# chenhonghua/MVIP-NeRF

Hardware: AMD Instinct MI355X
Metric: rays_per_sec (coarse+fine, 64+128 samples, 504x378) (higher is better)
Workload: dtype f32; 1 GPU; render 378x504 frame, 64 coarse + 128 fine samples, 8x256 MLP x2, lindisp, white_bkgd, test-mode kwargs (BASELINE configs[1] geometry at the metric resolution); points_per_ray=192, chunk=32768, parallelism=rays x1 (whole frames on one GPU)

## Files before the change

### include/mvip_nerf.h

```cpp
#ifndef MVIP_NERF_H
#define MVIP_NERF_H

#include <stdint.h>

#ifdef __cplusplus
extern "C" {
#endif

#define MVIP_OK        0
#define MVIP_EINVAL   -1
#define MVIP_ELAUNCH  -2
#define MVIP_EUNSUP   -3

#define MVIP_ABI_VERSION 5

int         mvip_abi_version(void);
int         mvip_build_is_experiment(void);
const char *mvip_strerror(int code);
const char *mvip_last_hip_error(void);
int         mvip_device_info(int *n_cu, int *lds_bytes, char *arch_out, int arch_cap);

int mvip_get_rays(const float *c2w, int H, int W, float focal, int y0, int x0, int h, int w,
                  float *rays_o, float *rays_d, void *stream);

// ... 24 lines not shown
                                      float *raw, void *stream);
int mvip_mlp_forward_rays_stash_f16x3_w16(const float *image, const float *rows, const float *z, int64_t B, int S,
                                          float *raw, float *stash, void *stream);

int mvip_mlp_forward_rays(const float *packed, const float *rows, const float *z, int64_t B, int S,
                          float *raw, int precision, void *stream);

int mvip_mlp_forward_points(const float *packed, const float *pts, const float *dirs, int64_t P,
                            float *raw, int precision, void *stream);

int mvip_mlp_pack16(const float *const *params_host, const float *packed, float *packed16, void *stream);
int mvip_mlp_forward_rays16(const float *packed16, const float *rows, const float *z, int64_t B, int S,
                            float *raw, void *stream);
int mvip_mlp_forward_points16(const float *packed16, const float *pts, const float *dirs, int64_t P,
                              float *raw, void *stream);
int mvip_mlp_encode16_probe(const float *pts, const float *dirs, int64_t P, float *out_old, float *out_new, void *stream);

int64_t mvip_mlp_packed_fold_floats(void);
int mvip_mlp_fold_pack16(const float *const *params_host, float *packed16_ext, void *stream);
int mvip_mlp_forward_rays16_fold(const float *packed16_ext, const float *rows, const float *z, int64_t B, int S,
                                 float *raw, void *stream);
int mvip_mlp_forward_points16_fold(const float *packed16_ext, const float *pts, const float *dirs, int64_t P,
                                   float *raw, void *stream);

int mvip_render_coarse_fused(const float *packed16, const float *rows, int64_t B, const float *t_vals, int lindisp,
                             const float *t_rand, const float *noise, const float *u, int u_is_row, int Nf, int flags,
                             float *rgb0, float *disp0, float *acc0, float *depth0, float *weights0, float *alpha0,
                             float *z_merged, float *z_std, void *stream);
int mvip_render_fine_fused(const float *packed16, const float *rows, const float *z, int64_t B, const float *noise,
                           int flags, float *raw, float *rgb, float *disp, float *acc, float *depth, float *weights,
                           float *alpha, void *stream);
int mvip_render_coarse_fused_fold(const float *packed16_ext, const float *rows, int64_t B, const float *t_vals, int lindisp,
                                  const float *t_rand, const float *noise, const float *u, int u_is_row, int Nf, int flags,
                                  float *rgb0, float *disp0, float *acc0, float *depth0, float *weights0, float *alpha0,
                                  float *z_merged, float *z_std, void *stream);
int mvip_render_fine_fused_fold(const float *packed16_ext, const float *rows, const float *z, int64_t B, const float *noise,
                                int flags, float *raw, float *rgb, float *disp, float *acc, float *depth, float *weights,
                                float *alpha, void *stream);

int64_t mvip_mlp_backward_workspace_bytes(int64_t tile_points);
int mvip_mlp_backward_rays(const float *packed, const float *rows, const float *z, int64_t B, int S,
                           const float *d_raw, float *const *grads_host, void *workspace,
                           int64_t tile_points, int precision, void *stream);
int mvip_mlp_backward_points(const float *packed, const float *pts, const float *dirs, int64_t P,
                             const float *d_raw, float *const *grads_host, void *workspace,
                             int64_t tile_points, int precision, void *stream);
int64_t mvip_mlp_stash_floats(int64_t P);
int mvip_mlp_forward_rays_stash(const float *packed, const float *rows, const float *z, int64_t B,
                                int S, float *raw, float *stash, int precision, void *stream);
int mvip_mlp_forward_points_stash(const float *packed, const float *pts, const float *dirs, int64_t P,
                                  float *raw, float *stash, int precision, void *stream);
int mvip_mlp_forward_rays_stash16(const float *packed16, const float *rows, const float *z, int64_t B, int S,
                                  float *raw, float *stash, void *stream);
int mvip_mlp_backward_stash(const float *packed, const float *stash, int64_t P, const float *d_raw,
                            float *const *grads_host, void *workspace, int64_t tile_points,
                            int precision, void *stream);
int mvip_mlp_unpack_grads(const float *grad_packed, float *const *grads_host, int accumulate,
                          void *stream);

#define MVIP_COMP_WHITE   1
#define MVIP_COMP_DETACHW 2
// ... 255 lines not shown
```

### mvip_nerf_amd/_lib.py

```python
import ctypes
import os

import torch

_HERE = os.path.dirname(os.path.abspath(__file__))
LIB_PATH = os.environ.get('MVIP_LIB_PATH') or os.path.join(_HERE, 'lib', 'libmvipnerf.so')

_c_f = ctypes.c_void_p
_i64 = ctypes.c_int64
_int = ctypes.c_int
_flt = ctypes.c_float

_SIGNATURES = {
    'mvip_abi_version': (_int, []),
    'mvip_build_is_experiment': (_int, []),
    'mvip_strerror': (ctypes.c_char_p, [_int]),
    'mvip_last_hip_error': (ctypes.c_char_p, []),
    'mvip_device_info': (_int, [ctypes.POINTER(_int), ctypes.POINTER(_int), ctypes.c_char_p, _int]),
    'mvip_get_rays': (_int, [_c_f, _int, _int, _flt, _int, _int, _int, _int, _c_f, _c_f, _c_f]),
    'mvip_ray_rows': (_int, [_c_f, _c_f, _c_f, _flt, _flt, _i64, _c_f, _c_f]),
    'mvip_ray_rows_from_pose': (_int, [_c_f, _int, _int, _flt, _flt, _flt, _c_f, _i64, _c_f, _c_f]),
    'mvip_stratified_z': (_int, [_c_f, _int, _i64, _int, _c_f, _int, _c_f, _c_f, _c_f]),
    'mvip_posenc': (_int, [_c_f, _i64, _int, _c_f, _c_f]),
    'mvip_mlp_packed_floats': (_i64, []),
# ... 2 lines not shown
    'mvip_mlp_forward_rays_f16x3': (_int, [_c_f, _c_f, _c_f, _i64, _int, _c_f, _c_f]),
    'mvip_mlp_forward_points_f16x3': (_int, [_c_f, _c_f, _c_f, _i64, _c_f, _c_f]),
    'mvip_mlp_pack_f16x3_w16': (_int, [ctypes.POINTER(ctypes.c_void_p), _c_f, _c_f, _c_f]),
    'mvip_mlp_forward_rays_f16x3_w16': (_int, [_c_f, _c_f, _c_f, _i64, _int, _c_f, _c_f]),
    'mvip_mlp_forward_points_f16x3_w16': (_int, [_c_f, _c_f, _c_f, _i64, _c_f, _c_f]),
    'mvip_mlp_forward_rays_stash_f16x3_w16': (_int, [_c_f, _c_f, _c_f, _i64, _int, _c_f, _c_f, _c_f]),
    'mvip_mlp_forward_rays': (_int, [_c_f, _c_f, _c_f, _i64, _int, _c_f, _int, _c_f]),
    'mvip_mlp_forward_points': (_int, [_c_f, _c_f, _c_f, _i64, _c_f, _int, _c_f]),
    'mvip_mlp_pack16': (_int, [ctypes.POINTER(ctypes.c_void_p), _c_f, _c_f, _c_f]),
    'mvip_mlp_forward_rays16': (_int, [_c_f, _c_f, _c_f, _i64, _int, _c_f, _c_f]),
    'mvip_mlp_forward_rays_stash16': (_int, [_c_f, _c_f, _c_f, _i64, _int, _c_f, _c_f, _c_f]),
    'mvip_mlp_forward_points16': (_int, [_c_f, _c_f, _c_f, _i64, _c_f, _c_f]),
    'mvip_mlp_encode16_probe': (_int, [_c_f, _c_f, _i64, _c_f, _c_f, _c_f]),
    'mvip_render_coarse_fused': (_int, [_c_f, _c_f, _i64, _c_f, _int, _c_f, _c_f, _c_f, _int, _int, _int, _c_f, _c_f, _c_f, _c_f,
                                        _c_f, _c_f, _c_f, _c_f, _c_f]),
    'mvip_render_fine_fused': (_int, [_c_f, _c_f, _c_f, _i64, _c_f, _int, _c_f, _c_f, _c_f, _c_f, _c_f, _c_f, _c_f, _c_f]),
    'mvip_mlp_packed_fold_floats': (_i64, []),
    'mvip_mlp_fold_pack16': (_int, [ctypes.POINTER(ctypes.c_void_p), _c_f, _c_f]),
    'mvip_mlp_forward_rays16_fold': (_int, [_c_f, _c_f, _c_f, _i64, _int, _c_f, _c_f]),
    'mvip_mlp_forward_points16_fold': (_int, [_c_f, _c_f, _c_f, _i64, _c_f, _c_f]),
    'mvip_render_coarse_fused_fold': (_int, [_c_f, _c_f, _i64, _c_f, _int, _c_f, _c_f, _c_f, _int, _int, _int, _c_f, _c_f, _c_f,
                                             _c_f, _c_f, _c_f, _c_f, _c_f, _c_f]),
    'mvip_render_fine_fused_fold': (_int, [_c_f, _c_f, _c_f, _i64, _c_f, _int, _c_f, _c_f, _c_f, _c_f, _c_f, _c_f, _c_f, _c_f]),
    'mvip_mlp_backward_workspace_bytes': (_i64, [_i64]),
    'mvip_mlp_backward_rays': (_int, [_c_f, _c_f, _c_f, _i64, _int, _c_f, ctypes.POINTER(ctypes.c_void_p), _c_f, _i64,
                                      _int, _c_f]),
    'mvip_mlp_backward_points': (_int, [_c_f, _c_f, _c_f, _i64, _c_f, ctypes.POINTER(ctypes.c_void_p), _c_f, _i64, _int,
                                        _c_f]),
    'mvip_mlp_stash_floats': (_i64, [_i64]),
    'mvip_mlp_forward_rays_stash': (_int, [_c_f, _c_f, _c_f, _i64, _int, _c_f, _c_f, _int, _c_f]),
    'mvip_mlp_forward_points_stash': (_int, [_c_f, _c_f, _c_f, _i64, _c_f, _c_f, _int, _c_f]),
    'mvip_mlp_backward_stash': (_int, [_c_f, _c_f, _i64, _c_f, ctypes.POINTER(ctypes.c_void_p), _c_f, _i64, _int, _c_f]),
    'mvip_mlp_unpack_grads': (_int, [_c_f, ctypes.POINTER(ctypes.c_void_p), _int, _c_f]),
    'mvip_composite_forward': (_int, [_c_f, _c_f, _c_f, _int, _c_f, _i64, _int, _int, _c_f, _c_f, _c_f, _c_f,
                                      _c_f, _c_f, _c_f]),
    'mvip_composite_backward': (_int, [_c_f, _c_f, _c_f, _int, _c_f, _i64, _int, _int, _c_f, _c_f, _c_f, _c_f,
                                       _c_f, _c_f, _c_f, _c_f]),
    'mvip_sample_pdf_merge': (_int, [_c_f, _c_f, _c_f, _int, _i64, _int, _int, _c_f, _c_f, _c_f, _c_f, _c_f,
                                     _c_f]),
    'mvip_sample_pdf': (_int, [_c_f, _c_f, _c_f, _int, _i64, _int, _int, _c_f, _c_f, _c_f, _c_f]),
    'mvip_depth2xyz': (_int, [_c_f, _int, _int, _flt, _flt, _flt, _flt, _c_f, _c_f]),
    'mvip_depth2xyz_backward': (_int, [_c_f, _int, _int, _flt, _flt, _flt, _flt, _c_f, _c_f]),
    'mvip_normal_fit_forward': (_int, [_c_f, _int, _int, _int, _c_f, _c_f, _c_f, _c_f]),
    'mvip_normal_fit_backward': (_int, [_c_f, _c_f, _c_f, _c_f, _int, _int, _int, _c_f, _c_f, _c_f]),
    'mvip_sds_add_noise': (_int, [_c_f, _c_f, _flt, _flt, _i64, _c_f, _c_f]),
    'mvip_sds_grad': (_int, [_c_f, _c_f, _c_f, _flt, _flt, _i64, _int, _c_f, _c_f]),
# ... 187 lines not shown
```

### mvip_nerf_amd/csrc/build.py

```python
import hashlib
import os
import shutil
import subprocess
import sys
from concurrent.futures import ThreadPoolExecutor

HERE = os.path.dirname(os.path.abspath(__file__))
PKG = os.path.dirname(HERE)
EXTRA_FLAGS = os.environ.get('MVIP_EXTRA_FLAGS', '').split()
EXPERIMENT = any(f.startswith('-DMVIP_EXPERIMENT') for f in EXTRA_FLAGS)
LIB_DIR = os.path.join(PKG, 'lib_experiment' if EXPERIMENT else 'lib')
OBJ_DIR = os.path.join(LIB_DIR, 'obj')
LIB_PATH = os.path.join(LIB_DIR, 'libmvipnerf.so')

SOURCES = ['api.hip', 'rays.hip', 'composite.hip', 'sample_pdf.hip', 'mlp_pack.hip', 'mlp_fwd.hip', 'mlp_fwd16.hip', 'mlp_fwd16_fold.hip', 'mlp_encode16_probe.hip', 'mlp_fwd_f16x3.hip', 'mlp_fwd16_f16x3.hip',
           'mlp_bwd.hip', 'mlp_bwd16.hip', 'mlp_bwd_f16x3.hip', 'normal_fit.hip', 'sds_elem.hip', 'group_norm.hip', 'conv3x3.hip', 'attention.hip', 'transformer.hip', 'hashgrid.hip', 'hashgrid_fused.hip', 'skinny_gemm.hip',
           'sd_sample.hip', 'mcubes.hip', 'occupancy.hip', 'region.hip', 'distortion.hip', 'harmonic.hip', 'warp.hip', 'ssim.hip', 'components.hip']
FLAGS = ['--offload-arch=gfx950', '-O3', '-std=c++17', '-fPIC', '-ffp-contract=off', '-Wall',
         '-Wno-unused-function'] + EXTRA_FLAGS


def _hipcc():
    for c in (os.environ.get('HIPCC'), shutil.which('hipcc'), '/opt/rocm/bin/hipcc'):
        if c and os.path.exists(c):
            return c
    raise RuntimeError('hipcc not found (need ROCm with gfx950 support)')


def _headers():
    hs = [os.path.join(HERE, f) for f in sorted(os.listdir(HERE)) if f.endswith('.h')]
    hs.append(os.path.join(os.path.dirname(PKG), 'include', 'mvip_nerf.h'))
    return hs


def _digest(path, header_blob):
    h = hashlib.sha256()
    h.update(open(path, 'rb').read())
    h.update(header_blob)
# ... 46 lines not shown
```

### mvip_nerf_amd/csrc/mlp_device16.h

```cpp
#pragma once
#include "common.h"
#include "mlp_layout.h"
#include "mlp_device.h"
#include <type_traits>

namespace mvip {
using namespace mlp;

namespace f16p {

typedef float f32x4 __attribute__((ext_vector_type(4)));
template <int V> using ic = std::integral_constant<int, V>;
template <int N, class F, int I = 0>
__device__ __forceinline__ void static_for(F &&f) {
    if constexpr (I < N) { f(ic<I>{}); static_for<N, F, I + 1>(static_cast<F &&>(f)); }
}

template <int C>
__device__ __forceinline__ float enc_channel(float x, float y, float z, int c) {
    const int m = c >= 3 ? c - 3 : 0;
    const int oct = m / 6, rem = m - 6 * oct;
    const int d = rem >= 3 ? rem - 3 : rem;
    const int dsel = c < 3 ? c : d;
    const float xv = dsel == 0 ? x : (dsel == 1 ? y : z);
// ... 47 lines not shown
    for (int t = 0; t < 4; ++t) emb[t] = ld4(row + (((4 * t + g) ^ n) << 2));
    __builtin_amdgcn_wave_barrier();
    row = stage + n * 32;
    const int nd = n >> 1;
    auto at_d = [&](int c) -> float & { return row[(((c >> 2) ^ nd) << 2) + (c & 3)]; };
    at_d(g < 3 ? g : 27) = g == 0 ? vx : (g == 1 ? vy : (g == 2 ? vz : 0.f));
    at_d(28 + g) = 0.f;
#pragma unroll
    for (int k = 0; k < 3; ++k) {
        const int j = g + 4 * k;
        const int oct = j / 3, axis = j - 3 * oct;
        const float xv = axis == 0 ? vx : (axis == 1 ? vy : vz);
        float s, c;
        sincosf(xv * __int_as_float((127 + oct) << 23), &s, &c);
        at_d(3 + 6 * oct + axis) = s;
        at_d(6 + 6 * oct + axis) = c;
    }
    __builtin_amdgcn_wave_barrier();
#pragma unroll
    for (int t = 0; t < 2; ++t) edir[t] = ld4(row + (((4 * t + g) ^ nd) << 2));
    __builtin_amdgcn_wave_barrier();
}

template <int NSLOT = NSLOT16, bool WRAP = false, bool FOLD = false>
struct Stream16T {
    const float *packed;
    float *lds;
    int wave, lane;
    int total_chunks = FOLD ? FOLD_TOTAL_CHUNKS : TOTAL_CHUNKS;
    lds_cfloat *lds_read = nullptr;
    static constexpr int nslot = NSLOT;
    static constexpr bool wrap = WRAP;
    __device__ __forceinline__ void issue_chunk(int g, int slot) const {
        if (WRAP && g >= total_chunks) g -= total_chunks;
        if (g < total_chunks) {
            const float *src = packed + (int64_t)g * CHUNK_FLOATS + wave * 512 + lane * 4;
            if constexpr (FOLD) { if (g >= FOLD_FIRST_CHUNK) src += FOLD_TAIL_A - FOLD_FIRST_CHUNK * CHUNK_FLOATS; }
            float *dst = lds + slot * CHUNK_FLOATS + wave * 512;
            glds<0>(src, dst);
            glds<1024>(src, dst);
        }
    }
    template <int BI>
    __device__ __forceinline__ f32x4 read_block() const {
        constexpr int off = ((BI / CHUNK_BLOCKS) % NSLOT) * CHUNK_FLOATS + (BI % CHUNK_BLOCKS) * BLOCK_FLOATS;
        if constexpr (WRAP) return ld4(lds_read + off + lane * 4);
        else return ld4(lds + off + lane * 4);
    }
};
using Stream16 = Stream16T<>;

__device__ __forceinline__ f32x4 mfma4(float a, float b, f32x4 c) {
    return __builtin_amdgcn_mfma_f32_16x16x4f32(a, b, c, 0, 0, 0);
}

struct NoPre16 { template <class T> __device__ __forceinline__ int operator()(T) const { return 0; } };
template <int BASE, int NTO, int NTI, bool LAST, bool HASB, class St, class Bias, class BSrc, class Pre, class Epi>
__device__ __forceinline__ void layer16x(const St &st, f32x4 &a, Bias bias, BSrc bsrc, Pre pre, Epi epi) {
    using PV = decltype(pre(ic<0>{}));
    f32x4 accs[2];
    PV pvs[2];
    static_for<NTO>([&](auto to_) {
        constexpr int TO = decltype(to_)::value;
        f32x4 &acc = accs[TO & 1];
        pvs[TO & 1] = pre(to_);
        if constexpr (HASB) acc = ld4(bias + 16 * TO + 4 * (st.lane >> 4));
        else acc = f32x4{0.f, 0.f, 0.f, 0.f};
        static_for<NTI>([&](auto ti_) {
            constexpr int TI = decltype(ti_)::value;
            constexpr int bi = BASE + TO * NTI + TI;
            constexpr bool last_block = LAST && (TO == NTO - 1) && (TI == NTI - 1);
            if constexpr (bi % CHUNK_BLOCKS == 0) st.issue_chunk(bi / CHUNK_BLOCKS + 2, (bi / CHUNK_BLOCKS + 2) % St::nslot);
            const f32x4 b = bsrc(ti_);
            acc = mfma4(a[0], b[0], acc);
            __builtin_amdgcn_sched_barrier(0);
            f32x4 an = a;
            if constexpr (!last_block) an = st.template read_block<bi + 1>();
            else if constexpr (St::wrap) an = st.template read_block<0>();
            __builtin_amdgcn_sched_barrier(0);
            acc = mfma4(a[1], b[1], acc);
            acc = mfma4(a[2], b[2], acc);
            acc = mfma4(a[3], b[3], acc);
            if constexpr (TI == NTI - 1) asm volatile("" : "+v"(acc));
#ifndef MVIP_EXPERIMENT_NO_BARRIER
            if constexpr (bi % CHUNK_BLOCKS == CHUNK_BLOCKS - 1) __syncthreads();
#endif
            a = an;
            if constexpr (TO > 0 && TI == 1) epi(ic<TO - 1>{}, accs[(TO - 1) & 1], pvs[(TO - 1) & 1]);
        });
    });
    epi(ic<NTO - 1>{}, accs[(NTO - 1) & 1], pvs[(NTO - 1) & 1]);
}
template <int BASE, int NTO, int NTI, bool LAST, class St, class Bias, class BSrc, class Epi>
__device__ __forceinline__ void layer16(const St &st, f32x4 &a, Bias bias, BSrc bsrc, Epi epi) {
    layer16x<BASE, NTO, NTI, LAST, true>(st, a, bias, bsrc, NoPre16{}, [&](auto to, const f32x4 &acc, int) { epi(to, acc); });
}

template <bool RELU>
__device__ __forceinline__ f32x4 act16(const f32x4 &acc) {
#ifdef MVIP_EXPERIMENT_NO_EPILOGUE
    return acc;
#endif
    f32x4 r;
#pragma unroll
    for (int i = 0; i < 4; ++i) {
        float v = acc[i];
        if (RELU) {
            const int bits = __builtin_bit_cast(int, v);
// ... 10 lines not shown
```

### mvip_nerf_amd/csrc/mlp_fwd16_kernel.h

```cpp
#pragma once
#include <stdlib.h>
#include "mlp_device16.h"
#include "rays_device.h"
#include "composite_device.h"
#include "sample_pdf_device.h"


namespace mvip {
using namespace mlp;

namespace f16p {

struct FuseArgs {
    const float *t_vals, *t_rand, *noise, *u;
    int u_is_row, lindisp, flags, Nf;
    float *rgb, *disp, *acc, *depth, *weights, *alpha, *z_merged, *z_std;
};

template <bool FROM_RAYS, bool STASH = false, int FUSE = 0, bool FOLD = false>
__global__ void __launch_bounds__(512, 2)
mlp_forward16_kernel(const float *__restrict__ packed, const float *__restrict__ in_a, const float *__restrict__ in_b,
                     int64_t P, int S, float *__restrict__ raw, float *__restrict__ stash = nullptr, int64_t n_pt = 0,
                     const FuseArgs fa = FuseArgs{}) {
    static_assert(!(STASH && FOLD), "the stash-writing forward needs the feature activations: it cannot fold");
    constexpr int NCHUNK = FOLD ? FOLD_TOTAL_CHUNKS : TOTAL_CHUNKS;
    __shared__ __attribute__((aligned(16))) float lds[LDS16_FLOATS];
    float *raw_s = lds + ((NCHUNK - 2) % NSLOT16) * CHUNK_FLOATS;
    const int lane = threadIdx.x & 63;
    const int wave = __builtin_amdgcn_readfirstlane(threadIdx.x >> 6);
    const int n = lane & 15, g = lane >> 4;
    int64_t p = (int64_t)blockIdx.x * WG_POINTS + wave * 16 + n;
    const bool live = p < P;
    if (!live) p = P - 1;

    Stream16T<NSLOT16, false, FOLD> st{packed, lds, wave, lane};
    constexpr int SEC_B_AT = FOLD ? FOLD_TAIL_B : SEC_A_FLOATS;
    for (int b = wave; b < SEC_B_FLOATS / BLOCK_FLOATS; b += 8)
        glds<0>(packed + SEC_B_AT + b * BLOCK_FLOATS + lane * 4, lds + RING16_FLOATS + b * BLOCK_FLOATS);
    st.issue_chunk(0, 0);
    st.issue_chunk(1, 1);

    float px, py, pz, vx, vy, vz;
    float zz = 0.f, zn = 0.f, nz = 0.f, dnorm = 0.f, tail_u = 2.f;
    int s_idx = 0;
    if constexpr (FROM_RAYS) {
        const int64_t ray = p / S;
        const float *row = in_a + ray * 11;
        s_idx = (int)(p - ray * S);
        if constexpr (FUSE == 1) {
            zz = stratified_point(row[6], row[7], fa.t_vals, s_idx, S, fa.lindisp, fa.t_rand ? fa.t_rand + p : nullptr);
            if (s_idx + 1 < S) zn = stratified_point(row[6], row[7], fa.t_vals, s_idx + 1, S, fa.lindisp, fa.t_rand ? fa.t_rand + p + 1 : nullptr);
        } else {
            zz = in_b[p];
            if constexpr (FUSE == 2) { if (s_idx + 1 < S) zn = in_b[p + 1]; }
        }
        px = row[0] + row[3] * zz; py = row[1] + row[4] * zz; pz = row[2] + row[5] * zz;
        vx = row[8]; vy = row[9]; vz = row[10];
        if constexpr (FUSE != 0) {
            constexpr int WPR_ = FUSE == 1 ? 4 : 8, SR_ = FUSE == 1 ? 64 : 128;
            dnorm = dir_norm(row);
            if (fa.noise) nz = fa.noise[p];
            if (FUSE == 1 && wave % WPR_ == 0) {
                const int64_t tray = (int64_t)blockIdx.x * (8 / WPR_) + wave / WPR_;
// ... 14 lines not shown
#pragma unroll
    for (int t = 0; t < 2; ++t)
#pragma unroll
        for (int i = 0; i < 4; ++i) edir[t][i] = vx * (float)(i + 1) + vy * (float)t;
#else
    encode16_wave(lds + 2 * CHUNK_FLOATS + wave * ENC_STAGE_FLOATS, lane, px, py, pz, vx, vy, vz, emb, edir);
#endif

    const int64_t pt_wave = (int64_t)blockIdx.x * 4 + (wave >> 1);
    const int stash_lane = (4 * g) * 32 + 16 * (wave & 1) + n;
    auto stash16 = [&](int t16, const f32x4 &t) {
        if constexpr (STASH) {
            float *q = stash + ((int64_t)(t16 >> 1) * n_pt + pt_wave) * 1024 + (t16 & 1) * 512 + stash_lane;
            q[0] = t[0]; q[32] = t[1]; q[64] = t[2]; q[96] = t[3];
        }
    };
#pragma unroll
    for (int t = 0; t < 4; ++t) stash16(2 * AT_EMB + t, emb[t]);
#pragma unroll
    for (int t = 0; t < 2; ++t) stash16(2 * AT_EDIR + t, edir[t]);

    __syncthreads();
    const float *sb = lds + RING16_FLOATS;
    f32x4 a = st.template read_block<0>();
    f32x4 h[16], o[16];

    layer16<OFF_L0, 16, NTI_L0, false>(st, a, sb + SB_BIAS, [&](auto ti) { return emb[ti.value]; },
        [&](auto to, const f32x4 &acc) { o[to.value] = act16<true>(acc); stash16(2 * AT_H + to.value, o[to.value]); });
#pragma unroll
    for (int t = 0; t < 16; ++t) h[t] = o[t];
    static_for<4>([&](auto li) {
        constexpr int l = 1 + decltype(li)::value;
        layer16<OFF_L1 + (l - 1) * LH_BLOCKS, 16, NTI_LH, false>(st, a, sb + SB_BIAS + l * 256, [&](auto ti) { return h[ti.value]; },
            [&](auto to, const f32x4 &acc) { o[to.value] = act16<true>(acc); stash16(2 * (AT_H + 8 * l) + to.value, o[to.value]); });
#pragma unroll
        for (int t = 0; t < 16; ++t) h[t] = o[t];
    });
    layer16<OFF_L5, 16, NTI_L5, false>(st, a, sb + SB_BIAS + 5 * 256,
        [&](auto ti) { if constexpr (ti.value < 4) return emb[ti.value]; else return h[ti.value - 4]; },
        [&](auto to, const f32x4 &acc) { o[to.value] = act16<true>(acc); stash16(2 * (AT_H + 40) + to.value, o[to.value]); });
#pragma unroll
    for (int t = 0; t < 16; ++t) h[t] = o[t];
    float sigma = 0.f;
    static_for<2>([&](auto li) {
        constexpr int l = 6 + decltype(li)::value;
        layer16<OFF_L6 + (l - 6) * LH_BLOCKS, 16, NTI_LH, false>(st, a, sb + SB_BIAS + l * 256, [&](auto ti) { return h[ti.value]; },
            [&](auto to, const f32x4 &acc) {
                o[to.value] = act16<true>(acc);
                stash16(2 * (AT_H + 8 * l) + to.value, o[to.value]);
                if constexpr (l == 7) {
                    const f32x4 w = *reinterpret_cast<const f32x4 *>(sb + SB_WALPHA + 16 * to.value + 4 * g);
#pragma unroll
                    for (int i = 0; i < 4; ++i) sigma = fmaf(w[i], o[to.value][i], sigma);
                }
            });
#pragma unroll
        for (int t = 0; t < 16; ++t) h[t] = o[t];
    });
    sigma += __shfl_xor(sigma, 16, 64);
    sigma += __shfl_xor(sigma, 32, 64);
    sigma += sb[SB_BALPHA];
    if constexpr (!FOLD)
        layer16<OFF_FEAT, 16, NTI_LH, false>(st, a, sb + SB_BFEAT, [&](auto ti) { return h[ti.value]; },
            [&](auto to, const f32x4 &acc) { o[to.value] = act16<false>(acc); stash16(2 * AT_FEAT + to.value, o[to.value]); });
    float r0 = 0.f, r1 = 0.f, r2 = 0.f;
    layer16<FOLD ? OFF_FEAT : OFF_VIEWS, 8, NTI_LV, true>(st, a, sb + (FOLD ? SB_BFOLD : SB_BVIEWS),
        [&](auto ti) {
            if constexpr (ti.value >= 16) return edir[ti.value - 16];
            else if constexpr (FOLD) return h[ti.value];
            else return o[ti.value];
        },
        [&](auto to, const f32x4 &acc) {
            const f32x4 v = act16<true>(acc);
            stash16(2 * AT_V + to.value, v);
            const f32x4 w0 = *reinterpret_cast<const f32x4 *>(sb + SB_WRGB + 16 * to.value + 4 * g);
            const f32x4 w1 = *reinterpret_cast<const f32x4 *>(sb + SB_WRGB + 128 + 16 * to.value + 4 * g);
            const f32x4 w2 = *reinterpret_cast<const f32x4 *>(sb + SB_WRGB + 256 + 16 * to.value + 4 * g);
#pragma unroll
            for (int i = 0; i < 4; ++i) {
                r0 = fmaf(w0[i], v[i], r0);
                r1 = fmaf(w1[i], v[i], r1);
                r2 = fmaf(w2[i], v[i], r2);
            }
        });
    r0 += __shfl_xor(r0, 16, 64); r1 += __shfl_xor(r1, 16, 64); r2 += __shfl_xor(r2, 16, 64);
    r0 += __shfl_xor(r0, 32, 64); r1 += __shfl_xor(r1, 32, 64); r2 += __shfl_xor(r2, 32, 64);
    const float4 out4 = make_float4(r0 + sb[SB_BRGB], r1 + sb[SB_BRGB + 1], r2 + sb[SB_BRGB + 2], sigma);
    if (live && g == 0 && raw) reinterpret_cast<float4 *>(raw)[p] = out4;
    if constexpr (FUSE != 0) {
        float *terms_s = raw_s, *z_s = raw_s + WG_POINTS * 4;
        {
            const float rc = g == 1 ? out4.x : (g == 2 ? out4.y : out4.z);
            const float x = g == 0 ? comp_neg_exponent(out4.w + nz, comp_dist(zz, zn, s_idx == S - 1, dnorm)) : -rc;
            const float e = expf(x);
            terms_s[(wave * 16 + n) * 4 + g] = g == 0 ? e : comp_sigmoid_from_exp(e);
            if (g == 0) z_s[wave * 16 + n] = zz;
        }
        __syncthreads();
        constexpr int RAYS = FUSE == 1 ? 2 : 1, WPR = 8 / RAYS, SR = WG_POINTS / RAYS;
        if (wave % WPR != 0) return;
#ifdef MVIP_EXPERIMENT_NO_FUSE_TAIL
        return;
#endif
        const int64_t ray = (int64_t)blockIdx.x * RAYS + wave / WPR;
        if (ray * SR >= P) return;
        constexpr int IT = SR / 64;
        RayState<IT> stt;
        float sums[5];
        ray_forward_terms<IT>(terms_s + (wave / WPR) * SR * 4, z_s + (wave / WPR) * SR, stt, sums);
        composite_store<IT>(stt, sums, ray, SR, fa.flags, fa.rgb, fa.disp, fa.acc, fa.depth, fa.weights, fa.alpha);
        if constexpr (FUSE == 1) {
            float zc[1] = {stt.z[0]}, wts[1], uu[1] = {tail_u};
            const float wn = __shfl_down(stt.w[0], 1, 64);
            wts[0] = lane < SR - 2 ? wn : 0.f;
            sample_merge_ray<1>(zc, wts, uu, ray, SR, fa.Nf, nullptr, fa.z_merged, fa.z_std, nullptr, nullptr);
        }
    }
}

struct ParamPtrsC16 { const float *p[P_COUNT]; };

}
}

namespace mvip {
namespace f16p {

template <bool FOLD>
static int forward_rays16(const float *packed16, const float *rows, const float *z, int64_t B, int S, float *raw, void *stream) {
    if (B < 0 || S <= 0) return MVIP_EINVAL;
    if (B == 0) return MVIP_OK;
    if (!packed16 || !rows || !z || !raw) return MVIP_EINVAL;
    const int64_t P = B * S;
    const int64_t tiles = (P + WG_POINTS - 1) / WG_POINTS;
    hipLaunchKernelGGL((mlp_forward16_kernel<true, false, 0, FOLD>), dim3((unsigned)tiles), dim3(512), 0,
                       as_stream(stream), packed16, rows, z, P, S, raw);
    return check_launch();
}

template <bool FOLD>
static int forward_points16(const float *packed16, const float *pts, const float *dirs, int64_t P, float *raw, void *stream) {
    if (P < 0) return MVIP_EINVAL;
    if (P == 0) return MVIP_OK;
    if (!packed16 || !pts || !dirs || !raw) return MVIP_EINVAL;
    hipLaunchKernelGGL((mlp_forward16_kernel<false, false, 0, FOLD>), dim3((unsigned)((P + WG_POINTS - 1) / WG_POINTS)), dim3(512), 0,
                       as_stream(stream), packed16, pts, dirs, P, 1, raw);
    return check_launch();
}

template <bool FOLD>
static int render_coarse_fused(const float *packed16, const float *rows, int64_t B, const float *t_vals, int lindisp,
                               const float *t_rand, const float *noise, const float *u, int u_is_row, int Nf, int flags,
                               float *rgb0, float *disp0, float *acc0, float *depth0, float *weights0, float *alpha0,
                               float *z_merged, float *z_std, void *stream) {
    if (B < 0 || Nf < 1 || Nf > 64) return MVIP_EINVAL;
    if (B == 0) return MVIP_OK;
    if (!packed16 || !rows || !t_vals || !u || !rgb0 || !disp0 || !acc0 || !z_merged || !z_std) return MVIP_EINVAL;
    FuseArgs fa;
    fa.t_vals = t_vals; fa.t_rand = t_rand; fa.noise = noise; fa.u = u; fa.u_is_row = u_is_row; fa.lindisp = lindisp;
    fa.flags = flags; fa.Nf = Nf;
    fa.rgb = rgb0; fa.disp = disp0; fa.acc = acc0; fa.depth = depth0; fa.weights = weights0; fa.alpha = alpha0;
    fa.z_merged = z_merged; fa.z_std = z_std;
    const int64_t P = B * 64;
    hipLaunchKernelGGL((mlp_forward16_kernel<true, false, 1, FOLD>), dim3((unsigned)((P + WG_POINTS - 1) / WG_POINTS)), dim3(512), 0,
                       as_stream(stream), packed16, rows, (const float *)nullptr, P, 64, (float *)nullptr, (float *)nullptr,
                       (int64_t)0, fa);
    return check_launch();
}

template <bool FOLD>
static int render_fine_fused(const float *packed16, const float *rows, const float *z, int64_t B, const float *noise,
                             int flags, float *raw, float *rgb, float *disp, float *acc, float *depth, float *weights,
                             float *alpha, void *stream) {
    if (B < 0) return MVIP_EINVAL;
    if (B == 0) return MVIP_OK;
    if (!packed16 || !rows || !z || !rgb || !disp || !acc || !depth || !weights) return MVIP_EINVAL;
    FuseArgs fa;
    fa.t_vals = nullptr; fa.t_rand = nullptr; fa.noise = noise; fa.u = nullptr; fa.u_is_row = 0; fa.lindisp = 0;
    fa.flags = flags; fa.Nf = 0;
    fa.rgb = rgb; fa.disp = disp; fa.acc = acc; fa.depth = depth; fa.weights = weights; fa.alpha = alpha;
    fa.z_merged = nullptr; fa.z_std = nullptr;
    const int64_t P = B * 128;
    hipLaunchKernelGGL((mlp_forward16_kernel<true, false, 2, FOLD>), dim3((unsigned)(P / WG_POINTS)), dim3(512), 0, as_stream(stream),
                       packed16, rows, z, P, 128, raw, (float *)nullptr, (int64_t)0, fa);
    return check_launch();
}

}
}
```

### mvip_nerf_amd/ops.py

```python
import weakref

import torch

from . import _lib
from ._lib import ptr, stream, call

_F32 = torch.float32


def _f32c(t):
    if t.dtype != _F32:
        t = t.float()
    return t if t.is_contiguous() else t.contiguous()



def get_rays(H, W, focal, c2w, patch=None):
    c = _f32c(c2w[:3, :4])
    y0, x0, h, w = (0, 0, H, W) if patch is None else [int(v) for v in patch]
    ro = torch.empty((h, w, 3), device=c.device, dtype=_F32)
    rd = torch.empty_like(ro)
    call('mvip_get_rays', ptr(c), int(H), int(W), float(focal), y0, x0, h, w, ptr(ro), ptr(rd), stream())
    return ro, rd

# ... 83 lines not shown


def mlp_pack16(params, packed_f32, fold=True):
    ps = [_f32c(p.detach()) for p in params]
    img = torch.empty(packed_fold_floats(), device=ps[0].device, dtype=_F32)
    call('mvip_mlp_pack16', _lib.ptr_array(ps), ptr(packed_f32), ptr(img), stream())
    if fold:
        call('mvip_mlp_fold_pack16', _lib.ptr_array(ps), ptr(img), stream())
    return img


def mlp_fold_pack16(params, img):
    if img.numel() != packed_fold_floats():
        raise _lib.MvipError('mlp_fold_pack16 needs the extended image of mlp_pack16')
    ps = [_f32c(p.detach()) for p in params]
    call('mvip_mlp_fold_pack16', _lib.ptr_array(ps), ptr(img), stream())
    return img


def plain16(img):
    return img[:packed_floats()]


def _fold16(packed16):
    n = packed16.numel()
    if n == packed_fold_floats():
        return '_fold'
    if n != packed_floats():
        raise _lib.MvipError(f'not an image of mlp_pack16: {n} floats')
    return ''


def mlp_pack_f16x3(params, packed_f32):
    ps = [_f32c(p.detach()) for p in params]
    img = torch.empty(packed_floats(), device=ps[0].device, dtype=_F32)
    call('mvip_mlp_pack_f16x3', _lib.ptr_array(ps), ptr(img), ptr(packed_f32), stream())
    return img


def mlp_pack_f16x3_w16(params, packed_f32):
    ps = [_f32c(p.detach()) for p in params]
    img = torch.empty(packed_floats(), device=ps[0].device, dtype=_F32)
    call('mvip_mlp_pack_f16x3_w16', _lib.ptr_array(ps), ptr(packed_f32), ptr(img), stream())
    return img


def mlp_unpack_grads(grad_packed, like):
    grads = [torch.empty(shp, device=grad_packed.device, dtype=_F32) for shp in PARAM_SHAPES]
    call('mvip_mlp_unpack_grads', ptr(grad_packed), _lib.ptr_array(grads), 0, stream())
    return grads
# ... 1837 lines not shown
```

Baseline: 714,300 rays/s.

## Stagger wave halves in folded MLP kernel to desynchronize weight-chunk barriers

Splits the eight waves of each workgroup into early and late groups. The late group places its chunk barrier and next-chunk issue at the middle of each chunk, prefetches one extra chunk ahead, and raises its scheduling priority. The aim is to keep the two halves out of phase so MFMA work from one half overlaps the LDS weight streaming and barrier waits of the other. It is enabled by default for folded inference launches through an environment flag. Risks are extra register or LDS-slot pressure from the deeper prefetch and code growth from instantiating the network twice.

```diff
diff --git a/include/mvip_nerf.h b/include/mvip_nerf.h
--- a/include/mvip_nerf.h
+++ b/include/mvip_nerf.h
@@ -70,6 +70,10 @@
                                  float *raw, void *stream);
 int mvip_mlp_forward_points16_fold(const float *packed16_ext, const float *pts, const float *dirs, int64_t P,
                                    float *raw, void *stream);
+int mvip_mlp_forward_rays16_fold_stagger(const float *packed16_ext, const float *rows, const float *z, int64_t B, int S,
+                                         float *raw, void *stream);
+int mvip_mlp_forward_points16_fold_stagger(const float *packed16_ext, const float *pts, const float *dirs, int64_t P,
+                                           float *raw, void *stream);
 
 int mvip_render_coarse_fused(const float *packed16, const float *rows, int64_t B, const float *t_vals, int lindisp,
                              const float *t_rand, const float *noise, const float *u, int u_is_row, int Nf, int flags,
@@ -85,6 +89,13 @@
 int mvip_render_fine_fused_fold(const float *packed16_ext, const float *rows, const float *z, int64_t B, const float *noise,
                                 int flags, float *raw, float *rgb, float *disp, float *acc, float *depth, float *weights,
                                 float *alpha, void *stream);
+int mvip_render_coarse_fused_fold_stagger(const float *packed16_ext, const float *rows, int64_t B, const float *t_vals,
+                                          int lindisp, const float *t_rand, const float *noise, const float *u, int u_is_row,
+                                          int Nf, int flags, float *rgb0, float *disp0, float *acc0, float *depth0,
+                                          float *weights0, float *alpha0, float *z_merged, float *z_std, void *stream);
+int mvip_render_fine_fused_fold_stagger(const float *packed16_ext, const float *rows, const float *z, int64_t B,
+                                        const float *noise, int flags, float *raw, float *rgb, float *disp, float *acc,
+                                        float *depth, float *weights, float *alpha, void *stream);
 
 int64_t mvip_mlp_backward_workspace_bytes(int64_t tile_points);
 int mvip_mlp_backward_rays(const float *packed, const float *rows, const float *z, int64_t B, int S,
diff --git a/mvip_nerf_amd/_lib.py b/mvip_nerf_amd/_lib.py
--- a/mvip_nerf_amd/_lib.py
+++ b/mvip_nerf_amd/_lib.py
@@ -48,6 +48,12 @@
     'mvip_render_coarse_fused_fold': (_int, [_c_f, _c_f, _i64, _c_f, _int, _c_f, _c_f, _c_f, _int, _int, _int, _c_f, _c_f, _c_f,
                                              _c_f, _c_f, _c_f, _c_f, _c_f, _c_f]),
     'mvip_render_fine_fused_fold': (_int, [_c_f, _c_f, _c_f, _i64, _c_f, _int, _c_f, _c_f, _c_f, _c_f, _c_f, _c_f, _c_f, _c_f]),
+    'mvip_mlp_forward_rays16_fold_stagger': (_int, [_c_f, _c_f, _c_f, _i64, _int, _c_f, _c_f]),
+    'mvip_mlp_forward_points16_fold_stagger': (_int, [_c_f, _c_f, _c_f, _i64, _c_f, _c_f]),
+    'mvip_render_coarse_fused_fold_stagger': (_int, [_c_f, _c_f, _i64, _c_f, _int, _c_f, _c_f, _c_f, _int, _int, _int, _c_f, _c_f,
+                                                     _c_f, _c_f, _c_f, _c_f, _c_f, _c_f, _c_f]),
+    'mvip_render_fine_fused_fold_stagger': (_int, [_c_f, _c_f, _c_f, _i64, _c_f, _int, _c_f, _c_f, _c_f, _c_f, _c_f, _c_f, _c_f,
+                                                   _c_f]),
     'mvip_mlp_backward_workspace_bytes': (_i64, [_i64]),
     'mvip_mlp_backward_rays': (_int, [_c_f, _c_f, _c_f, _i64, _int, _c_f, ctypes.POINTER(ctypes.c_void_p), _c_f, _i64,
                                       _int, _c_f]),
diff --git a/mvip_nerf_amd/csrc/build.py b/mvip_nerf_amd/csrc/build.py
--- a/mvip_nerf_amd/csrc/build.py
+++ b/mvip_nerf_amd/csrc/build.py
@@ -13,7 +13,7 @@
 OBJ_DIR = os.path.join(LIB_DIR, 'obj')
 LIB_PATH = os.path.join(LIB_DIR, 'libmvipnerf.so')
 
-SOURCES = ['api.hip', 'rays.hip', 'composite.hip', 'sample_pdf.hip', 'mlp_pack.hip', 'mlp_fwd.hip', 'mlp_fwd16.hip', 'mlp_fwd16_fold.hip', 'mlp_encode16_probe.hip', 'mlp_fwd_f16x3.hip', 'mlp_fwd16_f16x3.hip',
+SOURCES = ['api.hip', 'rays.hip', 'composite.hip', 'sample_pdf.hip', 'mlp_pack.hip', 'mlp_fwd.hip', 'mlp_fwd16.hip', 'mlp_fwd16_fold.hip', 'mlp_fwd16_stagger.hip', 'mlp_fwd16_stagger_fused.hip', 'mlp_encode16_probe.hip', 'mlp_fwd_f16x3.hip', 'mlp_fwd16_f16x3.hip',
            'mlp_bwd.hip', 'mlp_bwd16.hip', 'mlp_bwd_f16x3.hip', 'normal_fit.hip', 'sds_elem.hip', 'group_norm.hip', 'conv3x3.hip', 'attention.hip', 'transformer.hip', 'hashgrid.hip', 'hashgrid_fused.hip', 'skinny_gemm.hip',
            'sd_sample.hip', 'mcubes.hip', 'occupancy.hip', 'region.hip', 'distortion.hip', 'harmonic.hip', 'warp.hip', 'ssim.hip', 'components.hip']
 FLAGS = ['--offload-arch=gfx950', '-O3', '-std=c++17', '-fPIC', '-ffp-contract=off', '-Wall',
diff --git a/mvip_nerf_amd/csrc/mlp_device16.h b/mvip_nerf_amd/csrc/mlp_device16.h
--- a/mvip_nerf_amd/csrc/mlp_device16.h
+++ b/mvip_nerf_amd/csrc/mlp_device16.h
@@ -93,8 +93,9 @@
     __builtin_amdgcn_wave_barrier();
 }
 
-template <int NSLOT = NSLOT16, bool WRAP = false, bool FOLD = false>
+template <int NSLOT = NSLOT16, bool WRAP = false, bool FOLD = false, bool LATE = false>
 struct Stream16T {
+    static_assert(!(WRAP && LATE), "the persistent kernel is not staggered");
     const float *packed;
     float *lds;
     int wave, lane;
@@ -102,6 +103,10 @@
     lds_cfloat *lds_read = nullptr;
     static constexpr int nslot = NSLOT;
     static constexpr bool wrap = WRAP;
+    static constexpr bool late = LATE;
+    static constexpr int barrier_block = LATE ? CHUNK_BLOCKS / 2 - 1 : CHUNK_BLOCKS - 1;
+    static constexpr int issue_block = LATE ? CHUNK_BLOCKS / 2 : 0;
+    static constexpr int issue_ahead = LATE ? 3 : 2;
     __device__ __forceinline__ void issue_chunk(int g, int slot) const {
         if (WRAP && g >= total_chunks) g -= total_chunks;
         if (g < total_chunks) {
@@ -120,6 +125,18 @@
     }
 };
 using Stream16 = Stream16T<>;
+
+template <bool LATE>
+constexpr int chunk_barriers(int blocks) {
+    int n = 0;
+    for (int bi = 0; bi < blocks; ++bi) n += bi % CHUNK_BLOCKS == Stream16T<NSLOT16, false, false, LATE>::barrier_block;
+    return n;
+}
+static_assert(chunk_barriers<false>(TOTAL_BLOCKS) == TOTAL_CHUNKS && chunk_barriers<true>(TOTAL_BLOCKS) == TOTAL_CHUNKS,
+              "early and late waves meet at the same number of chunk barriers (plain stream)");
+static_assert(chunk_barriers<false>(FOLD_TOTAL_CHUNKS * CHUNK_BLOCKS) == FOLD_TOTAL_CHUNKS &&
+              chunk_barriers<true>(FOLD_TOTAL_CHUNKS * CHUNK_BLOCKS) == FOLD_TOTAL_CHUNKS,
+              "early and late waves meet at the same number of chunk barriers (folded stream)");
 
 __device__ __forceinline__ f32x4 mfma4(float a, float b, f32x4 c) {
     return __builtin_amdgcn_mfma_f32_16x16x4f32(a, b, c, 0, 0, 0);
@@ -141,7 +158,9 @@
             constexpr int TI = decltype(ti_)::value;
             constexpr int bi = BASE + TO * NTI + TI;
             constexpr bool last_block = LAST && (TO == NTO - 1) && (TI == NTI - 1);
-            if constexpr (bi % CHUNK_BLOCKS == 0) st.issue_chunk(bi / CHUNK_BLOCKS + 2, (bi / CHUNK_BLOCKS + 2) % St::nslot);
+            if constexpr (St::late && bi == 0) st.issue_chunk(2, 2 % St::nslot);
+            if constexpr (bi % CHUNK_BLOCKS == St::issue_block)
+                st.issue_chunk(bi / CHUNK_BLOCKS + St::issue_ahead, (bi / CHUNK_BLOCKS + St::issue_ahead) % St::nslot);
             const f32x4 b = bsrc(ti_);
             acc = mfma4(a[0], b[0], acc);
             __builtin_amdgcn_sched_barrier(0);
@@ -154,7 +173,7 @@
             acc = mfma4(a[3], b[3], acc);
             if constexpr (TI == NTI - 1) asm volatile("" : "+v"(acc));
 #ifndef MVIP_EXPERIMENT_NO_BARRIER
-            if constexpr (bi % CHUNK_BLOCKS == CHUNK_BLOCKS - 1) __syncthreads();
+            if constexpr (bi % CHUNK_BLOCKS == St::barrier_block) __syncthreads();
 #endif
             a = an;
             if constexpr (TO > 0 && TI == 1) epi(ic<TO - 1>{}, accs[(TO - 1) & 1], pvs[(TO - 1) & 1]);
diff --git a/mvip_nerf_amd/csrc/mlp_fwd16_kernel.h b/mvip_nerf_amd/csrc/mlp_fwd16_kernel.h
--- a/mvip_nerf_amd/csrc/mlp_fwd16_kernel.h
+++ b/mvip_nerf_amd/csrc/mlp_fwd16_kernel.h
@@ -17,12 +17,13 @@
     float *rgb, *disp, *acc, *depth, *weights, *alpha, *z_merged, *z_std;
 };
 
-template <bool FROM_RAYS, bool STASH = false, int FUSE = 0, bool FOLD = false>
+template <bool FROM_RAYS, bool STASH = false, int FUSE = 0, bool FOLD = false, bool STAGGER = false>
 __global__ void __launch_bounds__(512, 2)
 mlp_forward16_kernel(const float *__restrict__ packed, const float *__restrict__ in_a, const float *__restrict__ in_b,
                      int64_t P, int S, float *__restrict__ raw, float *__restrict__ stash = nullptr, int64_t n_pt = 0,
                      const FuseArgs fa = FuseArgs{}) {
     static_assert(!(STASH && FOLD), "the stash-writing forward needs the feature activations: it cannot fold");
+    static_assert(!STAGGER || (FOLD && !STASH), "only the folded inference launches are staggered");
     constexpr int NCHUNK = FOLD ? FOLD_TOTAL_CHUNKS : TOTAL_CHUNKS;
     __shared__ __attribute__((aligned(16))) float lds[LDS16_FLOATS];
     float *raw_s = lds + ((NCHUNK - 2) % NSLOT16) * CHUNK_FLOATS;
@@ -33,12 +34,12 @@
     const bool live = p < P;
     if (!live) p = P - 1;
 
-    Stream16T<NSLOT16, false, FOLD> st{packed, lds, wave, lane};
+    Stream16T<NSLOT16, false, FOLD> st0{packed, lds, wave, lane};
     constexpr int SEC_B_AT = FOLD ? FOLD_TAIL_B : SEC_A_FLOATS;
     for (int b = wave; b < SEC_B_FLOATS / BLOCK_FLOATS; b += 8)
         glds<0>(packed + SEC_B_AT + b * BLOCK_FLOATS + lane * 4, lds + RING16_FLOATS + b * BLOCK_FLOATS);
-    st.issue_chunk(0, 0);
-    st.issue_chunk(1, 1);
+    st0.issue_chunk(0, 0);
+    st0.issue_chunk(1, 1);
 
     float px, py, pz, vx, vy, vz;
     float zz = 0.f, zn = 0.f, nz = 0.f, dnorm = 0.f, tail_u = 2.f;
@@ -99,67 +100,86 @@
 
     __syncthreads();
     const float *sb = lds + RING16_FLOATS;
-    f32x4 a = st.template read_block<0>();
     f32x4 h[16], o[16];
-
-    layer16<OFF_L0, 16, NTI_L0, false>(st, a, sb + SB_BIAS, [&](auto ti) { return emb[ti.value]; },
-        [&](auto to, const f32x4 &acc) { o[to.value] = act16<true>(acc); stash16(2 * AT_H + to.value, o[to.value]); });
-#pragma unroll
-    for (int t = 0; t < 16; ++t) h[t] = o[t];
-    static_for<4>([&](auto li) {
-        constexpr int l = 1 + decltype(li)::value;
-        layer16<OFF_L1 + (l - 1) * LH_BLOCKS, 16, NTI_LH, false>(st, a, sb + SB_BIAS + l * 256, [&](auto ti) { return h[ti.value]; },
-            [&](auto to, const f32x4 &acc) { o[to.value] = act16<true>(acc); stash16(2 * (AT_H + 8 * l) + to.value, o[to.value]); });
+    float sigma = 0.f, r0 = 0.f, r1 = 0.f, r2 = 0.f;
+    auto network = [&](auto late_) {
+        Stream16T<NSLOT16, false, FOLD, decltype(late_)::value> st{packed, lds, wave, lane};
+#ifndef MVIP_STAGGER_NO_SETPRIO
+        if constexpr (decltype(late_)::value) __builtin_amdgcn_s_setprio(1);
+#endif
+        f32x4 a = st.template read_block<0>();
+
+        layer16<OFF_L0, 16, NTI_L0, false>(st, a, sb + SB_BIAS, [&](auto ti) { return emb[ti.value]; },
+            [&](auto to, const f32x4 &acc) { o[to.value] = act16<true>(acc); stash16(2 * AT_H + to.value, o[to.value]); });
 #pragma unroll
         for (int t = 0; t < 16; ++t) h[t] = o[t];
-    });
-    layer16<OFF_L5, 16, NTI_L5, false>(st, a, sb + SB_BIAS + 5 * 256,
-        [&](auto ti) { if constexpr (ti.value < 4) return emb[ti.value]; else return h[ti.value - 4]; },
-        [&](auto to, const f32x4 &acc) { o[to.value] = act16<true>(acc); stash16(2 * (AT_H + 40) + to.value, o[to.value]); });
-#pragma unroll
-    for (int t = 0; t < 16; ++t) h[t] = o[t];
-    float sigma = 0.f;
-    static_for<2>([&](auto li) {
-        constexpr int l = 6 + decltype(li)::value;
-        layer16<OFF_L6 + (l - 6) * LH_BLOCKS, 16, NTI_LH, false>(st, a, sb + SB_BIAS + l * 256, [&](auto ti) { return h[ti.value]; },
+        static_for<4>([&](auto li) {
+            constexpr int l = 1 + decltype(li)::value;
+            layer16<OFF_L1 + (l - 1) * LH_BLOCKS, 16, NTI_LH, false>(st, a, sb + SB_BIAS + l * 256, [&](auto ti) { return h[ti.value]; },
+                [&](auto to, const f32x4 &acc) { o[to.value] = act16<true>(acc); stash16(2 * (AT_H + 8 * l) + to.value, o[to.value]); });
+#pragma unroll
+            for (int t = 0; t < 16; ++t) h[t] = o[t];
+        });
+        layer16<OFF_L5, 16, NTI_L5, false>(st, a, sb + SB_BIAS + 5 * 256,
+            [&](auto ti) { if constexpr (ti.value < 4) return emb[ti.value]; else return h[ti.value - 4]; },
+            [&](auto to, const f32x4 &acc) { o[to.value] = act16<true>(acc); stash16(2 * (AT_H + 40) + to.value, o[to.value]); });
+#pragma unroll
+        for (int t = 0; t < 16; ++t) h[t] = o[t];
+        static_for<2>([&](auto li) {
+            constexpr int l = 6 + decltype(li)::value;
+            layer16<OFF_L6 + (l - 6) * LH_BLOCKS, 16, NTI_LH, false>(st, a, sb + SB_BIAS + l * 256, [&](auto ti) { return h[ti.value]; },
+                [&](auto to, const f32x4 &acc) {
+                    o[to.value] = act16<true>(acc);
+                    stash16(2 * (AT_H + 8 * l) + to.value, o[to.value]);
+                    if constexpr (l == 7) {
+                        const f32x4 w = *reinterpret_cast<const f32x4 *>(sb + SB_WALPHA + 16 * to.value + 4 * g);
+#pragma unroll
+                        for (int i = 0; i < 4; ++i) sigma = fmaf(w[i], o[to.value][i], sigma);
+                    }
+                });
+#pragma unroll
+            for (int t = 0; t < 16; ++t) h[t] = o[t];
+        });
+        sigma += __shfl_xor(sigma, 16, 64);
+        sigma += __shfl_xor(sigma, 32, 64);
+        sigma += sb[SB_BALPHA];
+        if constexpr (!FOLD)
+            layer16<OFF_FEAT, 16, NTI_LH, false>(st, a, sb + SB_BFEAT, [&](auto ti) { return h[ti.value]; },
+                [&](auto to, const f32x4 &acc) { o[to.value] = act16<false>(acc); stash16(2 * AT_FEAT + to.value, o[to.value]); });
+        layer16<FOLD ? OFF_FEAT : OFF_VIEWS, 8, NTI_LV, true>(st, a, sb + (FOLD ? SB_BFOLD : SB_BVIEWS),
+            [&](auto ti) {
+                if constexpr (ti.value >= 16) return edir[ti.value - 16];
+                else if constexpr (FOLD) return h[ti.value];
+                else return o[ti.value];
+            },
             [&](auto to, const f32x4 &acc) {
-                o[to.value] = act16<true>(acc);
-                stash16(2 * (AT_H + 8 * l) + to.value, o[to.value]);
-                if constexpr (l == 7) {
-                    const f32x4 w = *reinterpret_cast<const f32x4 *>(sb + SB_WALPHA + 16 * to.value + 4 * g);
-#pragma unroll
-                    for (int i = 0; i < 4; ++i) sigma = fmaf(w[i], o[to.value][i], sigma);
+                const f32x4 v = act16<true>(acc);
+                stash16(2 * AT_V + to.value, v);
+                const f32x4 w0 = *reinterpret_cast<const f32x4 *>(sb + SB_WRGB + 16 * to.value + 4 * g);
+                const f32x4 w1 = *reinterpret_cast<const f32x4 *>(sb + SB_WRGB + 128 + 16 * to.value + 4 * g);
+                const f32x4 w2 = *reinterpret_cast<const f32x4 *>(sb + SB_WRGB + 256 + 16 * to.value + 4 * g);
+#pragma unroll
+                for (int i = 0; i < 4; ++i) {
+                    r0 = fmaf(w0[i], v[i], r0);
+                    r1 = fmaf(w1[i], v[i], r1);
+                    r2 = fmaf(w2[i], v[i], r2);
                 }
             });
-#pragma unroll
-        for (int t = 0; t < 16; ++t) h[t] = o[t];
-    });
-    sigma += __shfl_xor(sigma, 16, 64);
-    sigma += __shfl_xor(sigma, 32, 64);
-    sigma += sb[SB_BALPHA];
-    if constexpr (!FOLD)
-        layer16<OFF_FEAT, 16, NTI_LH, false>(st, a, sb + SB_BFEAT, [&](auto ti) { return h[ti.value]; },
-            [&](auto to, const f32x4 &acc) { o[to.value] = act16<false>(acc); stash16(2 * AT_FEAT + to.value, o[to.value]); });
-    float r0 = 0.f, r1 = 0.f, r2 = 0.f;
-    layer16<FOLD ? OFF_FEAT : OFF_VIEWS, 8, NTI_LV, true>(st, a, sb + (FOLD ? SB_BFOLD : SB_BVIEWS),
-        [&](auto ti) {
-            if constexpr (ti.value >= 16) return edir[ti.value - 16];
-            else if constexpr (FOLD) return h[ti.value];
-            else return o[ti.value];
-        },
-        [&](auto to, const f32x4 &acc) {
-            const f32x4 v = act16<true>(acc);
-            stash16(2 * AT_V + to.value, v);
-            const f32x4 w0 = *reinterpret_cast<const f32x4 *>(sb + SB_WRGB + 16 * to.value + 4 * g);
-            const f32x4 w1 = *reinterpret_cast<const f32x4 *>(sb + SB_WRGB + 128 + 16 * to.value + 4 * g);
-            const f32x4 w2 = *reinterpret_cast<const f32x4 *>(sb + SB_WRGB + 256 + 16 * to.value + 4 * g);
-#pragma unroll
-            for (int i = 0; i < 4; ++i) {
-                r0 = fmaf(w0[i], v[i], r0);
-                r1 = fmaf(w1[i], v[i], r1);
-                r2 = fmaf(w2[i], v[i], r2);
-            }
-        });
+#ifndef MVIP_STAGGER_NO_SETPRIO
+        if constexpr (decltype(late_)::value) __builtin_amdgcn_s_setprio(0);
+#endif
+    };
+    if constexpr (STAGGER) {
+#ifdef MVIP_STAGGER_PARITY
+        const bool early = (wave & 1) == 0;
+#else
+        const bool early = wave < 4;
+#endif
+        if (early) network(std::false_type{});
+        else network(std::true_type{});
+    } else {
+        network(std::false_type{});
+    }
     r0 += __shfl_xor(r0, 16, 64); r1 += __shfl_xor(r1, 16, 64); r2 += __shfl_xor(r2, 16, 64);
     r0 += __shfl_xor(r0, 32, 64); r1 += __shfl_xor(r1, 32, 64); r2 += __shfl_xor(r2, 32, 64);
     const float4 out4 = make_float4(r0 + sb[SB_BRGB], r1 + sb[SB_BRGB + 1], r2 + sb[SB_BRGB + 2], sigma);
@@ -203,29 +223,29 @@
 namespace mvip {
 namespace f16p {
 
-template <bool FOLD>
+template <bool FOLD, bool STAGGER = false>
 static int forward_rays16(const float *packed16, const float *rows, const float *z, int64_t B, int S, float *raw, void *stream) {
     if (B < 0 || S <= 0) return MVIP_EINVAL;
     if (B == 0) return MVIP_OK;
     if (!packed16 || !rows || !z || !raw) return MVIP_EINVAL;
     const int64_t P = B * S;
     const int64_t tiles = (P + WG_POINTS - 1) / WG_POINTS;
-    hipLaunchKernelGGL((mlp_forward16_kernel<true, false, 0, FOLD>), dim3((unsigned)tiles), dim3(512), 0,
+    hipLaunchKernelGGL((mlp_forward16_kernel<true, false, 0, FOLD, STAGGER>), dim3((unsigned)tiles), dim3(512), 0,
                        as_stream(stream), packed16, rows, z, P, S, raw);
     return check_launch();
 }
 
-template <bool FOLD>
+template <bool FOLD, bool STAGGER = false>
 static int forward_points16(const float *packed16, const float *pts, const float *dirs, int64_t P, float *raw, void *stream) {
     if (P < 0) return MVIP_EINVAL;
     if (P == 0) return MVIP_OK;
     if (!packed16 || !pts || !dirs || !raw) return MVIP_EINVAL;
-    hipLaunchKernelGGL((mlp_forward16_kernel<false, false, 0, FOLD>), dim3((unsigned)((P + WG_POINTS - 1) / WG_POINTS)), dim3(512), 0,
+    hipLaunchKernelGGL((mlp_forward16_kernel<false, false, 0, FOLD, STAGGER>), dim3((unsigned)((P + WG_POINTS - 1) / WG_POINTS)), dim3(512), 0,
                        as_stream(stream), packed16, pts, dirs, P, 1, raw);
     return check_launch();
 }
 
-template <bool FOLD>
+template <bool FOLD, bool STAGGER = false>
 static int render_coarse_fused(const float *packed16, const float *rows, int64_t B, const float *t_vals, int lindisp,
                                const float *t_rand, const float *noise, const float *u, int u_is_row, int Nf, int flags,
                                float *rgb0, float *disp0, float *acc0, float *depth0, float *weights0, float *alpha0,
@@ -239,13 +259,13 @@
     fa.rgb = rgb0; fa.disp = disp0; fa.acc = acc0; fa.depth = depth0; fa.weights = weights0; fa.alpha = alpha0;
     fa.z_merged = z_merged; fa.z_std = z_std;
     const int64_t P = B * 64;
-    hipLaunchKernelGGL((mlp_forward16_kernel<true, false, 1, FOLD>), dim3((unsigned)((P + WG_POINTS - 1) / WG_POINTS)), dim3(512), 0,
+    hipLaunchKernelGGL((mlp_forward16_kernel<true, false, 1, FOLD, STAGGER>), dim3((unsigned)((P + WG_POINTS - 1) / WG_POINTS)), dim3(512), 0,
                        as_stream(stream), packed16, rows, (const float *)nullptr, P, 64, (float *)nullptr, (float *)nullptr,
                        (int64_t)0, fa);
     return check_launch();
 }
 
-template <bool FOLD>
+template <bool FOLD, bool STAGGER = false>
 static int render_fine_fused(const float *packed16, const float *rows, const float *z, int64_t B, const float *noise,
                              int flags, float *raw, float *rgb, float *disp, float *acc, float *depth, float *weights,
                              float *alpha, void *stream) {
@@ -258,7 +278,7 @@
     fa.rgb = rgb; fa.disp = disp; fa.acc = acc; fa.depth = depth; fa.weights = weights; fa.alpha = alpha;
     fa.z_merged = nullptr; fa.z_std = nullptr;
     const int64_t P = B * 128;
-    hipLaunchKernelGGL((mlp_forward16_kernel<true, false, 2, FOLD>), dim3((unsigned)(P / WG_POINTS)), dim3(512), 0, as_stream(stream),
+    hipLaunchKernelGGL((mlp_forward16_kernel<true, false, 2, FOLD, STAGGER>), dim3((unsigned)(P / WG_POINTS)), dim3(512), 0, as_stream(stream),
                        packed16, rows, z, P, 128, raw, (float *)nullptr, (int64_t)0, fa);
     return check_launch();
 }
diff --git a/mvip_nerf_amd/csrc/mlp_fwd16_stagger.hip b/mvip_nerf_amd/csrc/mlp_fwd16_stagger.hip
--- /dev/null
+++ b/mvip_nerf_amd/csrc/mlp_fwd16_stagger.hip
@@ -0,0 +1,14 @@
+#include "mlp_fwd16_kernel.h"
+
+using namespace mvip;
+using namespace mvip::f16p;
+
+extern "C" int mvip_mlp_forward_rays16_fold_stagger(const float *packed16_ext, const float *rows, const float *z, int64_t B,
+                                                    int S, float *raw, void *stream) {
+    return forward_rays16<true, true>(packed16_ext, rows, z, B, S, raw, stream);
+}
+
+extern "C" int mvip_mlp_forward_points16_fold_stagger(const float *packed16_ext, const float *pts, const float *dirs, int64_t P,
+                                                      float *raw, void *stream) {
+    return forward_points16<true, true>(packed16_ext, pts, dirs, P, raw, stream);
+}
diff --git a/mvip_nerf_amd/csrc/mlp_fwd16_stagger_fused.hip b/mvip_nerf_amd/csrc/mlp_fwd16_stagger_fused.hip
--- /dev/null
+++ b/mvip_nerf_amd/csrc/mlp_fwd16_stagger_fused.hip
@@ -0,0 +1,20 @@
+#include "mlp_fwd16_kernel.h"
+
+using namespace mvip;
+using namespace mvip::f16p;
+
+extern "C" int mvip_render_coarse_fused_fold_stagger(const float *packed16_ext, const float *rows, int64_t B,
+                                                     const float *t_vals, int lindisp, const float *t_rand, const float *noise,
+                                                     const float *u, int u_is_row, int Nf, int flags, float *rgb0, float *disp0,
+                                                     float *acc0, float *depth0, float *weights0, float *alpha0,
+                                                     float *z_merged, float *z_std, void *stream) {
+    return render_coarse_fused<true, true>(packed16_ext, rows, B, t_vals, lindisp, t_rand, noise, u, u_is_row, Nf, flags, rgb0,
+                                           disp0, acc0, depth0, weights0, alpha0, z_merged, z_std, stream);
+}
+
+extern "C" int mvip_render_fine_fused_fold_stagger(const float *packed16_ext, const float *rows, const float *z, int64_t B,
+                                                   const float *noise, int flags, float *raw, float *rgb, float *disp,
+                                                   float *acc, float *depth, float *weights, float *alpha, void *stream) {
+    return render_fine_fused<true, true>(packed16_ext, rows, z, B, noise, flags, raw, rgb, disp, acc, depth, weights, alpha,
+                                         stream);
+}
diff --git a/mvip_nerf_amd/ops.py b/mvip_nerf_amd/ops.py
--- a/mvip_nerf_amd/ops.py
+++ b/mvip_nerf_amd/ops.py
@@ -1,3 +1,4 @@
+import os
 import weakref
 
 import torch
@@ -129,10 +130,13 @@
     return img[:packed_floats()]
 
 
+STAGGER_INFERENCE = bool(int(os.environ.get('MVIP_STAGGER_INFERENCE', '1')))
+
+
 def _fold16(packed16):
     n = packed16.numel()
     if n == packed_fold_floats():
-        return '_fold'
+        return '_fold_stagger' if STAGGER_INFERENCE else '_fold'
     if n != packed_floats():
         raise _lib.MvipError(f'not an image of mlp_pack16: {n} floats')
     return ''
```

New measurement: 718,800 rays/s, median of 6. No clear change (+0.6%).
